# kyotovision-public/DRMNet

Measured on AMD Instinct MI355X. Metric: U-Net denoise steps/sec on 3x128x256 refmaps, higher is better.
Workload: dtype emulated fp32: f16 hi*hi + e4m3 cross terms (~15-bit products), fp32 acc; 1e-4 contract

## Files before the change

### drmnet_amd/_lib.py

```python
from __future__ import annotations

import ctypes as C
import os
from typing import Optional, Sequence

import torch

_HERE = os.path.dirname(os.path.abspath(__file__))
LIB_PATH = os.environ.get("DRM_LIB_PATH") or os.path.join(_HERE, "csrc", "libdrmnet_hip.so")
ABI_VERSION = 3
MAX_LEVELS = 8
LOSS_WORKSPACE_BYTES = 2048
DIFFUSION_LOSS_MAX_PARTS = 32
BRDF_ERROR_SUMS = 9
BRDF_ERROR_PARTS = 128


def diffusion_loss_workspace_bytes(B: int) -> int:
    return int(B) * DIFFUSION_LOSS_MAX_PARTS * 2 * 8


def brdf_error_workspace_bytes(C: int) -> int:
    return int(C) * BRDF_ERROR_PARTS * BRDF_ERROR_SUMS * 8


SYMBOLS = [
    "drm_abi_version", "drm_last_error",
    "drm_unet_create", "drm_unet_destroy", "drm_unet_param_count", "drm_unet_param_info", "drm_unet_load_params",
    "drm_unet_workspace_bytes", "drm_unet_forward",
    "drm_linear_forward", "drm_timestep_embedding", "drm_op_norm_act_conv", "drm_op_resblock", "drm_op_attention_block",
    "drm_drmnet_create", "drm_drmnet_destroy", "drm_drmnet_workspace_bytes", "drm_drmnet_set_batch_parts", "drm_drmnet_set_batch_part_min", "drm_drmnet_step", "drm_drmnet_sample",
    "drm_sampler_workspace_bytes", "drm_ddim_sample", "drm_ddim_sample_logged", "drm_ddpm_sample", "drm_ddim_sample_ex", "drm_ddpm_sample_ex", "drm_randn",
    "drm_profile_enable", "drm_profile_reset", "drm_profile_collect", "drm_unet_set_precision", "drm_set_op_precision",
    "drm_refmap_workspace_bytes", "drm_refmap_mask_make", "drm_erode_mask",
    "drm_unet_load_params_set", "drm_unet_use_set", "drm_set_graph_replay", "drm_set_upconv_split", "drm_graph_launches",
    "drm_map_chain", "drm_masked_log_range", "drm_luminance_scale", "drm_mirmap2envmap", "drm_hdr2ldr", "drm_resize", "drm_profile_variants",
    "drm_render_refmap", "drm_brdf_eval", "drm_render_refmap_views", "drm_validation_losses",
    "drm_render_refmap_lit", "drm_render_light_workspace_bytes",
    "drm_render_mesh_workspace_bytes", "drm_render_mesh",
    "drm_mesh_bvh_bytes", "drm_mesh_bvh_build", "drm_mesh_occluded", "drm_render_mesh_shadowed", "drm_render_mesh_lit",
    "drm_mesh_closest_hit", "drm_render_mesh_bounced",
    "drm_render_normals", "drm_image_from_refmap",
    "drm_brdf_to_merl", "drm_merl_eval", "drm_render_refmap_table", "drm_render_normals_table", "drm_brdf_error_sums",
    "drm_obs_forward_process", "drm_diffusion_losses",
    "drm_envmap2mirmap", "drm_rotate_envmap", "drm_mirimg2envmap", "drm_refmap2refimg",
]


class UNetDesc(C.Structure):
    _fields_ = [
# ... 118 lines not shown
    L.drm_ddpm_sample_ex.argtypes = [vp, fp, fp, fp, C.POINTER(C.c_float), i32, i32, fp, C.c_uint64, C.POINTER(SamplerOptions), i32, i32, i32, vp, C.c_size_t, vp]
    L.drm_randn.argtypes = [fp, C.c_size_t, C.c_uint64, C.c_uint64, vp]
    u8p = vp
    L.drm_refmap_workspace_bytes.argtypes = [C.c_int64, i32, C.c_float]
    L.drm_refmap_workspace_bytes.restype = C.c_size_t
    L.drm_refmap_mask_make.argtypes = [fp, fp, C.c_int64, i32, i32, C.c_float, i32, fp, u8p, vp, C.c_size_t, vp]
    L.drm_erode_mask.argtypes = [u8p, i32, i32, i32, u8p, vp]
    L.drm_unet_set_precision.argtypes = [vp, i32]
    L.drm_set_op_precision.argtypes = [i32]
    L.drm_profile_enable.argtypes = [i32]
    L.drm_profile_enable.restype = None
    L.drm_profile_reset.restype = None
    L.drm_profile_collect.argtypes = [C.POINTER(C.c_double), C.POINTER(C.c_double), C.POINTER(C.c_double), C.POINTER(C.c_int64)]
    L.drm_set_graph_replay.argtypes = [i32]
    L.drm_set_upconv_split.argtypes = [i32]
    L.drm_graph_launches.restype = C.c_int64
    L.drm_map_chain.argtypes = [fp, fp, C.c_int64, i32, C.POINTER(C.c_int32), C.POINTER(C.c_float), i32, fp, fp, fp, vp]
    L.drm_masked_log_range.argtypes = [fp, fp, i32, i32, i32, fp, fp, vp]
    L.drm_luminance_scale.argtypes = [fp, i32, i32, C.c_float, fp, vp]
    L.drm_mirmap2envmap.argtypes = [fp, fp, fp, i32, i32, i32, i32, i32, i32, i32, i32, vp]
    L.drm_hdr2ldr.argtypes = [fp, u8p, i32, C.c_float, C.c_float, fp, vp]
    L.drm_resize.argtypes = [fp, fp, i32, i32, i32, i32, i32, i32, vp]
    L.drm_profile_variants.argtypes = [C.c_char_p, C.c_size_t]
    L.drm_profile_variants.restype = C.c_size_t
    L.drm_render_refmap.argtypes = [fp, fp, fp, i32, i32, i32, i32, i32, i32, i32, vp]
    L.drm_brdf_eval.argtypes = [fp, i32, fp, fp, fp, fp, C.c_int64, vp]
    L.drm_render_refmap_views.argtypes = [fp, i32, fp, fp, fp, i32, i32, i32, i32, i32, i32, i32, vp]
    L.drm_render_refmap_lit.argtypes = [fp, i32, fp, fp, fp, i32, i32, i32, i32, i32, i32, i32, i32, vp, C.c_size_t, vp]
    L.drm_render_light_workspace_bytes.argtypes = [i32, i32, i32, i32]
    L.drm_render_light_workspace_bytes.restype = C.c_size_t
# ... 77 lines not shown
```

### drmnet_amd/csrc/abi.hip

```cpp
#include <atomic>
#include <cstring>
#include <memory>

#include "bvh.h"
#include "profiler.h"
#include "samplers.h"

using namespace drm;

struct drm_unet {
  UNet net;
};
struct drm_drmnet {
  DrmnetSampler s;
};

namespace {

int make_arena(Arena& ar, void* ws, size_t bytes, size_t need) {
  if (need == 0) return DRM_ERR_INVALID;
  if (bytes < need || ws == nullptr) {
    set_error("workspace too small: need " + std::to_string(need) + " bytes, got " + std::to_string(bytes));
    return DRM_ERR_WORKSPACE;
  }
// ... 409 lines not shown
    DRM_REQUIRE(precision_valid(precision),
                "precision must be 0 (fp32 MFMA), 1 (split fp16 x3), 2 (plain fp16 operands), 3 (split fp16 with fp8 cross terms) or 4 (plain bf16 operands)");
    g_op_precision.store(precision, std::memory_order_relaxed);
    return DRM_OK;
  });
}

int drm_set_upconv_split(int mode) {
  return guarded([&]() -> int {
    DRM_REQUIRE(mode >= 0 && mode <= 2, "upconv split mode: 0 = never, 1 = by the measured rule, 2 = wherever the form applies");
    set_upconv_split(mode);
    return DRM_OK;
  });
}

int drm_set_graph_replay(int on) {
  set_graph_replay(on != 0);
  return DRM_OK;
}
int64_t drm_graph_launches(void) { return (int64_t)graph_launches(); }

void drm_profile_enable(int on) { prof_enable(on); }
void drm_profile_reset(void) { prof_reset(); }
int drm_profile_collect(double* ms, double* flops, double* bytes, int64_t* launches) {
  return guarded([&]() -> int {
    DRM_REQUIRE(ms && flops && bytes && launches, "null argument");
    prof_collect(ms, flops, bytes, launches);
    return DRM_OK;
  });
}
// ... 279 lines not shown
```

### drmnet_amd/csrc/common.h

```cpp
#pragma once
#include <hip/hip_runtime.h>
#include <stdint.h>
#include <stdio.h>
#include <atomic>
#include <string>
#include "conv_forms.h"
#include "gn_fold.h"

namespace drm {

void set_error(const std::string& msg);
const char* last_error();

#define DRM_OK 0
#define DRM_ERR_INVALID 1
#define DRM_ERR_HIP 2
#define DRM_ERR_WORKSPACE 3
#define DRM_ERR_STATE 4

#define DRM_HIP_CHECK(expr)                                                                              \
  do {                                                                                                   \
    hipError_t _e = (expr);                                                                              \
    if (_e != hipSuccess) {                                                                              \
      ::drm::set_error(std::string(#expr) + " failed: " + hipGetErrorString(_e) + " at " + __FILE__ + ":" + \
// ... 37 lines not shown
struct XcdRange { int start, count; };
__host__ __device__ __forceinline__ XcdRange xcd_range(int total, int xcd) {
  const int q8 = total >> 3, r8 = total & 7;
  return {xcd < r8 ? xcd * (q8 + 1) : r8 * (q8 + 1) + (xcd - r8) * q8, q8 + (xcd < r8 ? 1 : 0)};
}


struct ConvArgs {
  const float* src0 = nullptr;
  const float* src1 = nullptr;
  int C0 = 0, C1 = 0, up0 = 0;
  int N = 0, H = 0, W = 0;
  const float* gn_scale = nullptr;
  const float* gn_shift = nullptr;
  int silu = 0;
  const float* w = nullptr;
  const float* bias = nullptr;
  int taps = 9;
  int Cout = 0;
  const float* emb = nullptr;
  int emb_stride = 0;
  const float* res = nullptr;
  float* out = nullptr;
  int out_nchw = 0, cout_valid = 0;
  int cin_real = 0;
  int ksplit = 1;
  size_t split_stride = 0;
  float* split_ws = nullptr;
  unsigned* tile_ticket = nullptr;
  int terms = 3;
// ... 26 lines not shown
struct ConvPlan {
  ConvKernel kernel = CONV_NONE;
  int terms = 0;
  ConvTile tile = TILE_128x32;
  int th = 0, tw = 0;
  bool ragged = false;
  int kc = 32;
  int ksplit = 1;
  SplitFinish finish = SPLIT_NONE;
  size_t tickets = 0;
  bool pool = false;
  bool gn_fold = false;
  bool split() const { return kernel == CONV_PIPELINE && terms != 0; }
};
ConvPlan plan_conv(const ConvArgs& a, int precision, bool want_pool = false, bool gn_foldable = false);
bool conv_split_weights(int precision, int cin);
int launch_conv(const ConvArgs& a, const ConvPlan& p, hipStream_t s);
template <int TAPS, int TERMS> int dispatch_s2(const ConvArgs& a, const ConvPlan& p, hipStream_t s);
int no_form(const ConvPlan& p);
size_t packed_conv_weight_split_floats(int taps, int CoutP, int CinP);
int launch_pack_conv_weight_split(const float* w, float* packed, float* scales, unsigned* scratch, int Cout, int Cin, int taps, int CoutP,
                                  int CinP, hipStream_t s, bool mx = false, bool bf16 = false);
enum Precision { PREC_FP32 = 0, PREC_F16X3 = 1, PREC_F16 = 2, PREC_F16MX = 3, PREC_BF16 = 4 };
inline bool precision_valid(int p) { return p >= PREC_FP32 && p <= PREC_BF16; }
inline int precision_terms(int p) { return p == PREC_F16 ? 1 : (p == PREC_BF16 ? 4 : (p == PREC_FP32 ? 0 : 3)); }
int launch_pack_conv_weight(const float* w, float* packed, int Cout, int Cin, int taps, int CoutP, int CinP, hipStream_t s);
int pack_conv_image(int precision, const float* w, float* packed, float* scale, unsigned* scratch, int Cout, int Cin, int taps, int CoutP, int CinP,
                    bool mx_site, hipStream_t s);
int launch_fold_upconv_weight(const float* w, float* wa, float* wb, int Cout, int C0, int C1, hipStream_t s);
int launch_fold_attn_params(const float* qkv_w, const float* qkv_b, const float* proj_w, const float* proj_b, float* w_out, float* b_out, int C,
// ... 139 lines not shown
```

### drmnet_amd/csrc/conv_plan.hip

```cpp
#include <algorithm>
#include "common.h"

namespace drm {

constexpr long long S2_MIN_WIDE_TILES = 176;
constexpr int GN_FOLD_MAX_N = 4;
bool conv_split_weights(int precision, int cin) { return precision != PREC_FP32 && cin % 32 == 0; }

static PixelTile conv_tile_family(int H, int W, bool pipeline) {
  auto area = [&](const PixelTile& f) { return (long long)((H + f.th - 1) / f.th * f.th) * ((W + f.tw - 1) / f.tw * f.tw); };
  const PixelTile* best = nullptr;
  for (const PixelTile& f : PIXEL_TILES)
    if (f.th * f.tw <= 128 && (!pipeline || pixel_tile_ragged(f.th, f.tw)) && (!best || area(f) < area(*best))) best = &f;
  return *best;
}

ConvPlan plan_conv(const ConvArgs& a, int precision, bool want_pool, bool gn_foldable) {
  ConvPlan p;
  const int Ctot = a.C0 + a.C1, hw = a.H * a.W;
  const bool split = precision != PREC_FP32, chunks = Ctot % 32 == 0 && a.C0 % 32 == 0;
  const long long rows = (long long)a.N * hw;
  auto wgs = [&](int bm, int bn) { return ((rows + bm - 1) / bm) * (a.Cout / bn); };
  if (a.w_img_stride_f4 != 0) {
    if (!split || a.H % 16 != 0 || a.W % 16 != 0 || a.Cout % 128 != 0 || Ctot % 128 != 0) return p;
// ... 41 lines not shown
  } else if (a.Cout % 64 == 0 && wgs(128, 64) >= 256) {
    tile(TILE_128x64, false);
  } else {
    tile(TILE_128x32, false);
  }
  p.ksplit = wide;
  if (wide == 1 && p.tile == TILE_128x32 && !a.out_nchw && a.w_img_stride_f4 == 0)
    p.ksplit = (int)std::max<long long>(std::min<long long>(std::min<long long>(8, Ctot / 32 / 4), 640 / std::max<long long>(wgs(128, 32), 1)), 1);
  if (p.ksplit > 1) {
    p.finish = (hw >= 128 && wide == 1) ? SPLIT_IN_LAUNCH : SPLIT_REDUCE;
    if (p.finish == SPLIT_IN_LAUNCH) p.tickets = ((size_t)a.N * hw / 128 + (size_t)hw / 16 + 2) * (size_t)(a.Cout / 32);
  }
  return p;
}

}
```

### drmnet_amd/csrc/conv_split2.hip

```cpp
#include <algorithm>
#include <utility>
#include <vector>
#include <cstdio>
#include <string>

#include "common.h"
#include "conv_epilogue.h"
#include "profiler.h"

#ifdef DRM_S2_STAMP
#define S2_STAMP(id)                                                                               \
  do {                                                                                             \
    if (stamp_on && stamp_n < 120) {                                                               \
      unsigned long long t_;                                                                       \
      __builtin_amdgcn_sched_barrier(0);                                                           \
      asm volatile("s_memtime %0\n\ts_waitcnt lgkmcnt(0)" : "=s"(t_)::"memory");                   \
      __builtin_amdgcn_sched_barrier(0);                                                           \
      if (lane == 0) {                                                                             \
        stamp_lds[(wave * 120 + stamp_n) * 2] = (unsigned)(id);                                    \
        stamp_lds[(wave * 120 + stamp_n) * 2 + 1] = (unsigned)t_;                                  \
      }                                                                                            \
      ++stamp_n;                                                                                   \
    }                                                                                              \
  } while (0)
// ... 126 lines not shown
               : "=&s"(keep)
               : "v"(voff), "s"(sbase), "s"(lds_dst)
               : "memory");
}
__device__ __forceinline__ void glds16(const void* gsrc, unsigned lds_dst) {
  unsigned keep;
  asm volatile("s_mov_b32 %0, m0\n\ts_mov_b32 m0, %2\n\ts_nop 0\n\tglobal_load_lds_dwordx4 %1, off\n\ts_mov_b32 m0, %0"
               : "=&s"(keep)
               : "v"(gsrc), "s"(lds_dst)
               : "memory");
}

__device__ __forceinline__ void gload16x2(f32x4& d0, f32x4& d1, const void* p) {
  asm volatile("global_load_dwordx4 %0, %2, off\n\tglobal_load_dwordx4 %1, %2, off offset:16" : "=&v"(d0), "=&v"(d1) : "v"(p) : "memory");
}
__device__ __forceinline__ void tie_regs(f32x4& x0, f32x4& x1) { asm volatile("" : "+v"(x0), "+v"(x1)::"memory"); }
__device__ __forceinline__ void tie_reg(f32x4& x) { asm volatile("" : "+v"(x)::"memory"); }

template <int... I, typename F>
__device__ __forceinline__ void static_for(std::integer_sequence<int, I...>, F&& f) {
  (f(std::integral_constant<int, I>{}), ...);
}

struct TilePos {
  int n0, ty0, tx0, co0;
  long long wofs;
};

template <int TAPS, int TH, int TW, int WM, int WN, int MT, int NT, int R, int TPS, int TERMS = 3, bool RAG = false, bool SK = false, bool POOL = false>
__global__ __launch_bounds__(WM* WN * 64, 2) void conv_split2_kernel(ConvArgs a) {
  using C = S2Cfg<TAPS, TH, TW, WM, WN, MT, NT, R, TPS, TERMS>;
  static_assert(!POOL || (C::SUB48 && C::TN == 1 && !RAG && !SK), "pooled output: one-image tiles of 4 x 8 patches");
  extern __shared__ float4 lds[];
  float4* As = lds;
  float4* Bs = lds + C::A_F4;
  double* lst = reinterpret_cast<double*>(lds + C::A_F4 + R * C::G_F4);
  [[maybe_unused]] double* lst2 = lst + C::TN * C::BN * 2;

#ifndef DRM_NO_KERNARG_TOUCH
  {
    typedef const __attribute__((address_space(4))) int* kptr_t;
    kptr_t ka = (kptr_t)__builtin_amdgcn_kernarg_segment_ptr();
    int touch = 0;
#pragma unroll
    for (int o = 0; o < (int)sizeof(ConvArgs); o += 64) touch ^= __builtin_nontemporal_load(ka + o / 4);
    asm volatile("" ::"s"(touch));
  }
// ... 232 lines not shown
  }
#pragma unroll
  for (int c = 0; c < NT; ++c) b_base[c] = (wn * NT + c) * 32 + r;

  f32x16 acc[MT][NT];
#pragma unroll
  for (int i = 0; i < MT; ++i)
#pragma unroll
    for (int c = 0; c < NT; ++c)
#pragma unroll
      for (int e = 0; e < 16; ++e) acc[i][c][e] = 0.f;

  const float inv_scale = a.w_inv_scale ? *a.w_inv_scale : 1.0f;
  constexpr int PPI = TH * TW;
  const bool st = a.stat_out != nullptr;
  if (st) {
    for (int k = tid; k < C::TN * C::BN * 2; k += C::NTHR) lst[k] = 0.0;
  }
  if constexpr (POOL) {
    for (int k = tid; k < C::TN * C::BN * 2; k += C::NTHR) lst2[k] = 0.0;
  }

  int gseq = 0;
  {
    int k2 = k_tile;
    TilePos tp = cur;
    int gi = 0;
#pragma unroll
    for (int G = 0; G < R - 1; ++G) {
      if (gi >= NGT) {
// ... 168 lines not shown
      gi = gi0 + (R - 1);
      co0 = cur.wofs;
      if (gi >= NGT) {
        gi -= NGT;
        if (gi >= NGT) gi %= NGT;
        co0 = nxt.wofs;
      }
    };
    auto issue_ahead = [&](int gi0) {
      int gi;
      long long co0;
      group_ahead(gi0, gi, co0);
      issue_G(gseq, gi, co0);
      ++gseq;
    };
    if constexpr (TAPS == 1) {
      for (int chunk = 0; chunk < nchunks; ++chunk) {
        const bool n1 = (chunk + 1 < nchunks) || has_next;
        const bool n2 = (chunk + 2 < nchunks) || (has_next && nchunks >= 2);
        auto side = [&]() {
          S2_STAMP(40);
          if (n1) {
            if (step == 0) wait_vmcnt<0>();
            else wait_vmcnt<C::G_PER>();
            S2_STAMP(41);
            store_A(As + ((step + 1) & 1) * C::A1_F4);
            S2_STAMP(42);
          }
          if (n2) {
            if (chunk + 2 < nchunks) load_A(cur, chunk + 2);
// ... 220 lines not shown
        const bool abl_noload = a.stamp_block & 0x200000;
#else
        constexpr bool abl_noload = false;
#endif
        if (a.res && first && !abl_noload) {
#pragma unroll
          for (int e = 0; e < 16; ++e) rv[e] = a.res[(pixb[e >> 2] + (e & 3)) * a.Cout + co];
        } else {
#pragma unroll
          for (int e = 0; e < 16; ++e) rv[e] = 0.f;
        }
        float s0 = 0.f, q0 = 0.f, s1 = 0.f, q1 = 0.f;
        float v[16];
#pragma unroll
        for (int e = 0; e < 16; ++e) {
          v[e] = epi_value(acc[i][c][e] * sv[e >> 2], bias, ev[e >> 2], rv[e]);
          acc[i][c][e] = 0.f;
        }
        const float p0 = okg[0] ? v[0] : (okg[1] ? v[4] : 0.f), p1 = okg[2] ? v[8] : (okg[3] ? v[12] : 0.f);
#pragma unroll
        for (int e = 0; e < 16; ++e) {
#ifdef DRM_S2_STAMP
          if (a.stamp_block & 0x100000) continue;
#endif
          if (okg[e >> 2]) {
            const float dv = v[e] - (e < 8 ? p0 : p1);
            if (e < 8) {
              s0 += dv;
              q0 += dv * dv;
            } else {
              s1 += dv;
// ... 255 lines not shown
    S2_STAMP(10);
    if (!has_next) break;
    k_tile += J;
    cur = nxt;
  }
  wait_vmcnt<0>();
#ifdef DRM_S2_STAMP
  if (a.stamp_out && (int)blockIdx.x == (a.stamp_block & 0xFFFF)) {
    asm volatile("s_waitcnt lgkmcnt(0)" ::: "memory");
    __builtin_amdgcn_s_barrier();
    for (int k = tid; k < C::NW * 240; k += C::NTHR) a.stamp_out[k] = stamp_lds[k];
  }
#endif
}

template <int TAPS, int TH, int TW, int WM, int WN, int MT, int NT, int R, int TPS, int TERMS = 3, bool RAG = false, bool SK = false, bool POOL = false>
static int launch_s2(const ConvArgs& a, hipStream_t s) {
  using C = S2Cfg<TAPS, TH, TW, WM, WN, MT, NT, R, TPS, TERMS>;
  constexpr auto kern = conv_split2_kernel<TAPS, TH, TW, WM, WN, MT, NT, R, TPS, TERMS, RAG, SK, POOL>;
  DRM_REQUIRE(RAG || (a.H % TH == 0 && a.W % TW == 0), "conv tile does not divide the map");
  DRM_REQUIRE(POOL == (a.pool_out != nullptr), "pooled output: only launches plan_conv pools");
  DRM_REQUIRE(!POOL || (a.pool_stat && a.stat_out && a.ksplit <= 1 && !a.out_nchw), "pooled output: needs both statistics tables, no split-K");
  if constexpr (TAPS == 4) {
    static_assert(!RAG && !SK && !POOL, "the parity form has no ragged, split-K or pooled instantiation");
    DRM_REQUIRE(!a.bias && !a.emb && !a.res && !a.stat_out && !a.out_nchw && a.ksplit <= 1 && !a.gnf.mom0 && !a.in_inv && a.w_img_stride_f4 == 0,
                "parity (4-tap) conv: weight un-scaling only -- no bias, emb, residual, statistics, split-K or GroupNorm fold");
    DRM_REQUIRE(a.C1 == 0 && !a.up0 && a.Cout % 4 == 0 && (a.Cout / 4) % C::BN == 0, "parity (4-tap) conv: one stored source, a Cout tile inside one parity");
  }
  const size_t lds_bytes = (size_t)(C::LDS_F4 + (POOL ? C::ST_F4 : 0)) * sizeof(float4);
  static_assert((C::LDS_F4 + (POOL ? C::ST_F4 : 0)) * 16 <= 160 * 1024, "LDS budget");
  const DeviceInfo* di = device_info();
  if (!di) return DRM_ERR_STATE;
  DRM_TRY(opt_in_lds<kern>(lds_bytes, di));
  const int groups = (a.N + C::TN - 1) / C::TN;
  const long long tiles = (long long)groups * ((a.H + TH - 1) / TH) * ((a.W + TW - 1) / TW) * (a.Cout / C::BN);
  DRM_REQUIRE(tiles > 0 && tiles < (1ll << 31), "conv grid size");
  const int per_cu = std::max(1, std::min((int)(di->lds_per_cu / lds_bytes), 8 / C::NW));
  long long grid = (long long)di->cus * per_cu;
  const int ngt = ((a.C0 + a.C1) / C::KC) * C::NG;
  const int ks = a.ksplit > 1 ? a.ksplit : 1;
  constexpr bool FUSE = SK;
  DRM_REQUIRE(ks == 1 || (!a.out_nchw && a.split_stride > 0 && a.w_img_stride_f4 == 0 && ((a.C0 + a.C1) / C::KC) / ks >= 1 && ks <= 8 &&
                          (a.split_ws ? (FUSE && a.tile_ticket != nullptr) : !a.stat_out)),
              "split-K launch contract");
  if (tiles < grid || ngt < R - 1 || (TAPS == 1 && ngt < 2) || ks > 1) grid = tiles;
  {
    prof_tag(a.N, a.H, a.W, a.C0 + a.C1, a.Cout);
    if (prof_enabled()) {
      static const std::string vname = [] {
        char b[192];
        snprintf(b, sizeof b, "void drm::conv_split2_kernel<%d, %d, %d, %d, %d, %d, %d, %d, %d, %d, %s, %s, %s>", TAPS, TH, TW, WM, WN, MT, NT, R, TPS, TERMS,
                 RAG ? "true" : "false", SK ? "true" : "false", POOL ? "true" : "false");
        return std::string(b);
      }();
      prof_variant(vname.c_str());
    }
    DRM_REQUIRE(a.w_img_stride_f4 == 0 || (C::TN == 1 && ks == 1), "per-image weights need one image per tile (H*W a multiple of the 256-pixel tile)");
    const ConvWork work = conv_work(a, TAPS);
    ProfScope ps(a.prof_kind == PROF_KINDS ? -1 : (a.prof_kind >= 0 ? a.prof_kind : (TAPS != 1 ? PROF_CONV3 : PROF_CONV1)), work.flops, work.bytes, s);
#ifdef DRM_S2_STAMP
    static const char* stamp_file = getenv("DRM_S2_STAMP_FILE");
    if (stamp_file && lds_bytes + 7680 <= di->lds_per_cu) {
      static unsigned* dbuf = nullptr;
      if (!dbuf) DRM_HIP_CHECK(hipMalloc(reinterpret_cast<void**>(&dbuf), 8192));
      DRM_HIP_CHECK(hipMemsetAsync(dbuf, 0, 8192, s));
      ConvArgs at = a;
// ... 18 lines not shown
      ConvArgs at = a;
      at.stamp_block = atoi(fl) & ~0xFFFF;
      hipLaunchKernelGGL(kern, dim3((unsigned)grid, (unsigned)ks), dim3(C::NTHR), lds_bytes, s, at);
    } else
#endif
    hipLaunchKernelGGL(kern, dim3((unsigned)grid, (unsigned)ks), dim3(C::NTHR), lds_bytes, s, a);
  }
  DRM_HIP_CHECK(hipGetLastError());
  return DRM_OK;
}

template <int TAPS, int TERMS, int TH, int TW, ConvTile T, bool RAG, bool SK, bool POOL>
static int launch_s2_form(const ConvArgs& a, const ConvPlan& p, hipStream_t s) {
  constexpr S2Form f = s2_form(TAPS, TERMS, TH, TW, T, RAG, SK, POOL);
  constexpr TileShape t = tile_shape(T);
  if constexpr (f.exists) return launch_s2<TAPS, TH, TW, t.wm, t.wn, t.mt, t.nt, f.ring, f.tps, TERMS, RAG, SK, POOL>(a, s);
  return no_form(p);
}

template <int TAPS, int TERMS, int TH, int TW, ConvTile T>
static int launch_s2_variant(const ConvArgs& a, const ConvPlan& p, hipStream_t s) {
  if (p.ragged) return launch_s2_form<TAPS, TERMS, TH, TW, T, true, false, false>(a, p, s);
  if (p.pool) return launch_s2_form<TAPS, TERMS, TH, TW, T, false, false, true>(a, p, s);
  if (p.finish == SPLIT_IN_LAUNCH) return launch_s2_form<TAPS, TERMS, TH, TW, T, false, true, false>(a, p, s);
  return launch_s2_form<TAPS, TERMS, TH, TW, T, false, false, false>(a, p, s);
}

template <int TAPS, int TERMS, int TH, int TW>
static int launch_s2_tile(const ConvArgs& a, const ConvPlan& p, hipStream_t s) {
#define DRM_X(name, wm, wn, mt, nt) if (p.tile == name) return launch_s2_variant<TAPS, TERMS, TH, TW, name>(a, p, s);
  DRM_CONV_TILES(DRM_X)
// ... 16 lines not shown
```

### drmnet_amd/csrc/engine.h

```cpp
#pragma once
#include <map>
#include <string>
#include <tuple>
#include <vector>

#include "../../include/drmnet_hip.h"
#include "common.h"

namespace drm {

struct Arena {
  char* base = nullptr;
  size_t cap = 0, off = 0, peak = 0;
  bool dry = false;
  bool failed = false;
  void* alloc_bytes(size_t bytes) {
    const size_t a = (off + 255) & ~size_t(255);
    off = a + bytes;
    if (off > peak) peak = off;
    if (dry) return nullptr;
    if (off > cap) {
      failed = true;
      return nullptr;
    }
// ... 127 lines not shown
  int dry_forward(int N, int H, int W, Arena& probe);
  ~UNet();
};

struct Ctx {
  Arena* ar;
  hipStream_t s;
  int N;
  int precision = PREC_FP32;
  bool dry() const { return ar->dry; }
  bool split() const { return precision == PREC_F16X3 || precision == PREC_F16 || precision == PREC_F16MX || precision == PREC_BF16; }
  int terms() const { return precision_terms(precision); }
};
Act new_act(Ctx& c, int C, int H, int W);
void set_upconv_split(int mode);
inline bool upconv_split_packable(int c0, int c1, int cout) { return c0 > 0 && c1 > 0 && c0 % 32 == 0 && c1 % 32 == 0 && cout % 32 == 0; }
int ensure_moments(Ctx& c, Act& a);
int expect_raw_sums(Ctx& c, Act& a);
int run_resblock(Ctx& c, const float* wbuf, const ResLayer& r, Act& x0, Act* x1, const float* emb_all, int emb_stride, Act& out, Act* pool = nullptr,
                 bool* pooled = nullptr);
int run_attention(Ctx& c, const float* wbuf, const AttnLayer& a, Act& x, Act& out);
int run_conv(Ctx& c, ConvArgs& a, const ConvPlan& p, const float* wbuf, size_t scale_off, Act* stats_for = nullptr);
int raw_input_guard(Ctx& c, ConvArgs& a, const ConvPlan& p, Act* x0, int lo0, int hi0, Act* x1, const unsigned* absmax_bits, int Ctab, int absmax_parts = 1);
int gn_params(Ctx& c, Act& x0, Act* x1, const float* gamma, const float* beta, float* scale, float* shift, ConvArgs* guard_for = nullptr,
              ConvArgs* fold_into = nullptr);

}
```

### drmnet_amd/csrc/engine.hip

```cpp
#include "engine.h"

#include <algorithm>
#include <atomic>
#include <deque>
#include <mutex>

namespace drm {

static thread_local std::string g_err;
void set_error(const std::string& msg) { g_err = msg; }
const char* last_error() { return g_err.c_str(); }

const DeviceInfo* device_info() {
  constexpr int MAX_DEV = 64;
  static DeviceInfo info[MAX_DEV];
  static std::atomic<int> state[MAX_DEV];
  int dev = 0;
  if (hipGetDevice(&dev) != hipSuccess || dev < 0 || dev >= MAX_DEV) {
    set_error("device_info: no current HIP device");
    return nullptr;
  }
  int st = state[dev].load(std::memory_order_acquire);
  if (st == 0) {
    static std::mutex mu;
// ... 405 lines not shown
  const int mode = g_upconv_split.load(std::memory_order_relaxed);
  if (mode == 0 || !r.up_c0 || !x0.up || !x1 || x0.C != r.up_c0 || !upconv_split_packable(x0.C, x1->C, r.cout)) return u;
  auto plain = [](const ConvPlan& p) { return p.kernel == CONV_PIPELINE && !p.ragged && p.ksplit == 1 && !p.gn_fold && !p.pool; };
  if (!plain(pa)) return u;
  u.a4.C0 = x0.C; u.a4.N = a.N; u.a4.H = a.H >> 1; u.a4.W = a.W >> 1; u.a4.taps = 4; u.a4.Cout = 4 * r.cout; u.a4.mx_site = 1;
  u.b9.C0 = x1->C; u.b9.N = a.N; u.b9.H = a.H; u.b9.W = a.W; u.b9.taps = 9; u.b9.Cout = r.cout; u.b9.mx_site = 1;
  u.p4 = plan_conv(u.a4, c.precision);
  u.p9 = plan_conv(u.b9, c.precision);
  if (!plain(u.p4) || !plain(u.p9)) return u;
  if (r.cout % tile_shape(u.p4.tile).bn() != 0) return u;
  if (mode == 1 && (u.p4.tile > TILE_256x128 || u.p9.tile > TILE_256x128)) return u;
  u.on = true;
  return u;
}

int run_resblock(Ctx& c, const float* Wb, const ResLayer& r, Act& x0, Act* x1, const float* emb_all, int emb_stride, Act& out, Act* pool, bool* pooled) {
  DRM_TRY(arena_ok(c));
  const int H = x0.H, W = x0.W;
  const int C0 = x0.C, C1 = x1 ? x1->C : 0;
  DRM_REQUIRE(C0 + C1 == r.cin, "resblock input channels");
  DRM_REQUIRE(!x1 || (x1->H == H && x1->W == W && !x1->up), "resblock skip tensor shape");
  DRM_REQUIRE(r.has_skip || (!x1 && !x0.up), "identity skip on a concatenated / upsampled input is not supported");
  const size_t mark = c.ar->mark();
  float* sc1 = c.ar->alloc<float>((size_t)c.N * r.cin);
  float* sh1 = c.ar->alloc<float>((size_t)c.N * r.cin);
  Act h1 = new_act(c, r.cout, H, W);
  float* sc2 = c.ar->alloc<float>((size_t)c.N * r.cout);
  float* sh2 = c.ar->alloc<float>((size_t)c.N * r.cout);
  ConvArgs k;
  ConvArgs a;
  a.src0 = x0.p; a.src1 = x1 ? x1->p : nullptr; a.C0 = C0; a.C1 = C1; a.up0 = x0.up;
  a.N = c.N; a.H = H; a.W = W; a.taps = 9; a.Cout = r.cout; a.mx_site = 1;
  const ConvPlan pa = plan_conv(a, c.precision, false, true);
  ConvPlan pk;
  if (r.has_skip) {
    k.C0 = C0; k.C1 = C1; k.N = c.N; k.H = H; k.W = W; k.taps = 1; k.Cout = r.cout;
    pk = plan_conv(k, c.precision);
  }
  DRM_TRY(gn_params(c, x0, x1, Wb + r.n1_w, Wb + r.n1_b, sc1, sh1, pk.split() ? &k : nullptr, pa.gn_fold ? &a : nullptr));
  splitk_workspace(c, a, pa);
  UpconvSplit up = plan_upconv_split(c, r, a, pa, x0, x1);
  if (up.on) {
    if (!c.dry()) {
      ConvArgs& a4 = up.a4;
      a4.src0 = x0.p; a4.gn_scale = sc1; a4.gn_shift = sh1; a4.gn_ld = r.cin; a4.silu = 1;
      a4.w = Wb + r.c1a_w; a4.out = h1.p;
      DRM_TRY(run_conv(c, a4, up.p4, Wb, r.c1a_s, nullptr));
      ConvArgs& b9 = up.b9;
      b9.src0 = x1->p; b9.gn_scale = sc1 + x0.C; b9.gn_shift = sh1 + x0.C; b9.gn_ld = r.cin; b9.silu = 1;
      b9.w = Wb + r.c1b_w; b9.bias = Wb + r.c1_b;
      b9.emb = emb_all ? emb_all + r.emb_off : nullptr; b9.emb_stride = emb_stride;
      b9.res = h1.p; b9.out = h1.p;
      DRM_TRY(run_conv(c, b9, up.p9, Wb, r.c1b_s, &h1));
    }
  } else if (!c.dry()) {
// ... 2 lines not shown
    a.emb = emb_all ? emb_all + r.emb_off : nullptr; a.emb_stride = emb_stride;
    a.out = h1.p;
    DRM_TRY(run_conv(c, a, pa, Wb, r.c1_s, &h1));
  }
  ConvArgs b;
  b.src0 = h1.p; b.C0 = r.cout; b.N = c.N; b.H = H; b.W = W; b.taps = 9; b.Cout = r.cout; b.mx_site = 1;
  const ConvPlan pb = plan_conv(b, c.precision, pool != nullptr, true);
  DRM_TRY(gn_params(c, h1, nullptr, Wb + r.n2_w, Wb + r.n2_b, sc2, sh2, nullptr, pb.gn_fold ? &b : nullptr));
  splitk_workspace(c, b, pb);
  if (pooled) *pooled = pb.pool;
  if (pb.pool) DRM_TRY(expect_raw_sums(c, *pool));
  if (r.has_skip) splitk_workspace(c, k, pk);
  if (!c.dry()) {
    const float* res = x0.p;
    if (r.has_skip) {
      k.src0 = x0.p; k.src1 = x1 ? x1->p : nullptr; k.up0 = x0.up;
      k.w = Wb + r.sk_w; k.bias = Wb + r.sk_b;
      k.out = out.p;
      DRM_TRY(run_conv(c, k, pk, Wb, r.sk_s, nullptr));
      res = out.p;
    }
    b.gn_scale = sc2; b.gn_shift = sh2; b.silu = 1;
    b.w = Wb + r.c2_w; b.bias = Wb + r.c2_b;
    b.res = res; b.out = out.p;
    if (pb.pool) {
      b.pool_out = pool->p;
      b.pool_stat = pool->mom;
    }
    DRM_TRY(run_conv(c, b, pb, Wb, r.c2_s, &out));
  }
  c.ar->release(mark);
  return DRM_OK;
}

// ... 222 lines not shown
```

### drmnet_amd/ops.py

```python
from __future__ import annotations

from typing import Optional, Sequence

import torch

from . import _lib


def set_precision(precision: str) -> None:
    modes = {"fp32": 0, "f16x3": 1, "f16": 2, "f16mx": 3, "bf16": 4}
    if precision not in modes:
        raise ValueError(f"precision must be one of {list(modes)}")
    _lib.check(_lib.lib().drm_set_op_precision(modes[precision]))


def set_graph_replay(on: bool) -> None:
    _lib.check(_lib.lib().drm_set_graph_replay(int(bool(on))))


def set_upconv_split(mode: int) -> None:
    _lib.check(_lib.lib().drm_set_upconv_split(int(mode)))


UPCONV_TAP_GROUPS = {0: {0: (0,), 1: (1, 2)}, 1: {0: (0, 1), 1: (2,)}}


def fold_upconv_weight(w: torch.Tensor, c0: int):
    cout = w.shape[0]
    w0 = w[:, :c0].double()
    wa = torch.zeros((4, cout, c0, 2, 2), dtype=torch.float64, device=w.device)
    for a in (0, 1):
        for b in (0, 1):
            for dy in (0, 1):
                for dx in (0, 1):
                    for ky in UPCONV_TAP_GROUPS[a][dy]:
                        for kx in UPCONV_TAP_GROUPS[b][dx]:
# ... 380 lines not shown
```

### include/drmnet_hip.h

```cpp
#ifndef DRMNET_HIP_H
#define DRMNET_HIP_H

#include <stddef.h>
#include <stdint.h>

#ifdef __cplusplus
extern "C" {
#endif

#define DRM_ABI_VERSION 3
#define DRM_MAX_LEVELS 8

int drm_abi_version(void);
const char* drm_last_error(void);

typedef struct drm_unet_desc {
  int32_t kind;
  int32_t in_channels;
  int32_t model_channels;
  int32_t out_channels;
  int32_t num_res_blocks;
  int32_t n_levels;
  int32_t channel_mult[DRM_MAX_LEVELS];
  int32_t n_attn;
// ... 87 lines not shown
  const float* dropout_keep;
} drm_sampler_options;

int drm_ddim_sample_ex(drm_unet* net, float* x, const float* cond, const int64_t* timesteps, const float* coef, int S, int num_steps,
                       const float* noise, uint64_t seed, const drm_sampler_options* opt, int log_every_t, float* log_x, float* log_pred_x0, int log_slots,
                       int32_t* n_logged, int N, int H, int W, void* workspace, size_t workspace_bytes, void* stream);
int drm_ddpm_sample_ex(drm_unet* net, float* x, float* pred_x0, const float* cond, const float* coef, int T_start, int clip_denoised,
                       const float* noise, uint64_t seed, const drm_sampler_options* opt, int N, int H, int W, void* workspace, size_t workspace_bytes,
                       void* stream);

size_t drm_sampler_workspace_bytes(const drm_unet* net, int N, int H, int W);

int drm_set_graph_replay(int on);

int drm_set_upconv_split(int mode);
int64_t drm_graph_launches(void);

#define DRM_PROFILE_KINDS 5
void drm_profile_enable(int on);
void drm_profile_reset(void);
int drm_profile_collect(double* ms, double* flops, double* bytes, int64_t* launches);
size_t drm_profile_variants(char* buf, size_t cap);

int drm_randn(float* out, size_t n, uint64_t seed, uint64_t offset, void* stream);

size_t drm_refmap_workspace_bytes(int64_t n, int res, float angle_threshold);
int drm_refmap_mask_make(const float* colors, const float* normals, int64_t n, int channels, int res, float angle_threshold, int min_points,
                         float* refmap, uint8_t* refmask, void* workspace, size_t workspace_bytes, void* stream);

int drm_erode_mask(const uint8_t* mask, int H, int W, int kernel_size, uint8_t* out, void* stream);
// ... 114 lines not shown
```

Baseline: 883.6.

## Compute upsampled half of decoder skip 1x1 conv at low resolution

For decoder resblocks whose 1x1 skip conv reads a nearest-upsampled source concatenated with a full-resolution source, the upsampled channels are now convolved at half resolution. Their raw accumulators are written to a slab. A second full-resolution 1x1 launch over the other source preloads those accumulators at the upsampled position before adding its own products and the bias. This removes the redundant three quarters of the MACs on the upsampled channels. In exchange it adds a kernel launch, a slab round trip through memory, and new template instantiations with a carried-accumulator path. It is on by default under a tile-size rule.

```diff
diff --git a/drmnet_amd/_lib.py b/drmnet_amd/_lib.py
--- a/drmnet_amd/_lib.py
+++ b/drmnet_amd/_lib.py
@@ -33,7 +33,7 @@
     "drm_sampler_workspace_bytes", "drm_ddim_sample", "drm_ddim_sample_logged", "drm_ddpm_sample", "drm_ddim_sample_ex", "drm_ddpm_sample_ex", "drm_randn",
     "drm_profile_enable", "drm_profile_reset", "drm_profile_collect", "drm_unet_set_precision", "drm_set_op_precision",
     "drm_refmap_workspace_bytes", "drm_refmap_mask_make", "drm_erode_mask",
-    "drm_unet_load_params_set", "drm_unet_use_set", "drm_set_graph_replay", "drm_set_upconv_split", "drm_graph_launches",
+    "drm_unet_load_params_set", "drm_unet_use_set", "drm_set_graph_replay", "drm_set_upconv_split", "drm_set_skip_lowres", "drm_graph_launches",
     "drm_map_chain", "drm_masked_log_range", "drm_luminance_scale", "drm_mirmap2envmap", "drm_hdr2ldr", "drm_resize", "drm_profile_variants",
     "drm_render_refmap", "drm_brdf_eval", "drm_render_refmap_views", "drm_validation_losses",
     "drm_render_refmap_lit", "drm_render_light_workspace_bytes",
@@ -182,6 +182,7 @@
     L.drm_profile_collect.argtypes = [C.POINTER(C.c_double), C.POINTER(C.c_double), C.POINTER(C.c_double), C.POINTER(C.c_int64)]
     L.drm_set_graph_replay.argtypes = [i32]
     L.drm_set_upconv_split.argtypes = [i32]
+    L.drm_set_skip_lowres.argtypes = [i32]
     L.drm_graph_launches.restype = C.c_int64
     L.drm_map_chain.argtypes = [fp, fp, C.c_int64, i32, C.POINTER(C.c_int32), C.POINTER(C.c_float), i32, fp, fp, fp, vp]
     L.drm_masked_log_range.argtypes = [fp, fp, i32, i32, i32, fp, fp, vp]
diff --git a/drmnet_amd/csrc/abi.hip b/drmnet_amd/csrc/abi.hip
--- a/drmnet_amd/csrc/abi.hip
+++ b/drmnet_amd/csrc/abi.hip
@@ -447,6 +447,14 @@
   });
 }
 
+int drm_set_skip_lowres(int mode) {
+  return guarded([&]() -> int {
+    DRM_REQUIRE(mode >= 0 && mode <= 2, "skip lowres mode: 0 = never, 1 = by the measured rule, 2 = wherever the form is legal");
+    set_skip_lowres(mode);
+    return DRM_OK;
+  });
+}
+
 int drm_set_graph_replay(int on) {
   set_graph_replay(on != 0);
   return DRM_OK;
diff --git a/drmnet_amd/csrc/common.h b/drmnet_amd/csrc/common.h
--- a/drmnet_amd/csrc/common.h
+++ b/drmnet_amd/csrc/common.h
@@ -75,6 +75,7 @@
   const float* gn_scale = nullptr;
   const float* gn_shift = nullptr;
   int silu = 0;
+  int acc_io = 0;
   const float* w = nullptr;
   const float* bias = nullptr;
   int taps = 9;
@@ -131,6 +132,12 @@
   bool split() const { return kernel == CONV_PIPELINE && terms != 0; }
 };
 ConvPlan plan_conv(const ConvArgs& a, int precision, bool want_pool = false, bool gn_foldable = false);
+struct SkipLowres {
+  bool on = false;
+  ConvArgs ka, kb;
+  ConvPlan pa, pb;
+};
+SkipLowres plan_skip_lowres(const ConvArgs& k, const ConvPlan& pk, int precision, int mode);
 bool conv_split_weights(int precision, int cin);
 int launch_conv(const ConvArgs& a, const ConvPlan& p, hipStream_t s);
 template <int TAPS, int TERMS> int dispatch_s2(const ConvArgs& a, const ConvPlan& p, hipStream_t s);
diff --git a/drmnet_amd/csrc/conv_plan.hip b/drmnet_amd/csrc/conv_plan.hip
--- a/drmnet_amd/csrc/conv_plan.hip
+++ b/drmnet_amd/csrc/conv_plan.hip
@@ -79,4 +79,23 @@
   return p;
 }
 
+static bool skip_lowres_rule(const SkipLowres& u) { return u.pa.tile <= TILE_256x128 && u.pb.tile <= TILE_256x128; }
+
+SkipLowres plan_skip_lowres(const ConvArgs& k, const ConvPlan& pk, int precision, int mode) {
+  SkipLowres u;
+  if (mode == 0 || k.taps != 1 || k.C0 <= 0 || k.C1 <= 0 || k.C0 % 32 != 0 || k.C1 % 32 != 0 || k.H % 2 != 0 || k.W % 2 != 0 || k.out_nchw ||
+      k.w_img_stride_f4 != 0)
+    return u;
+  auto plain = [](const ConvPlan& p) { return p.kernel == CONV_PIPELINE && !p.ragged && p.ksplit == 1 && !p.gn_fold && !p.pool; };
+  if (!plain(pk)) return u;
+  u.ka.C0 = k.C0; u.ka.N = k.N; u.ka.H = k.H >> 1; u.ka.W = k.W >> 1; u.ka.taps = 1; u.ka.Cout = k.Cout;
+  u.kb.C0 = k.C1; u.kb.N = k.N; u.kb.H = k.H; u.kb.W = k.W; u.kb.taps = 1; u.kb.Cout = k.Cout;
+  u.pa = plan_conv(u.ka, precision);
+  u.pb = plan_conv(u.kb, precision);
+  if (!plain(u.pa) || !plain(u.pb) || u.pa.terms != pk.terms || u.pb.terms != pk.terms) return u;
+  if (mode == 1 && !skip_lowres_rule(u)) return u;
+  u.on = true;
+  return u;
 }
+
+}
diff --git a/drmnet_amd/csrc/conv_split2.hip b/drmnet_amd/csrc/conv_split2.hip
--- a/drmnet_amd/csrc/conv_split2.hip
+++ b/drmnet_amd/csrc/conv_split2.hip
@@ -164,6 +164,7 @@
 __device__ __forceinline__ void gload16x2(f32x4& d0, f32x4& d1, const void* p) {
   asm volatile("global_load_dwordx4 %0, %2, off\n\tglobal_load_dwordx4 %1, %2, off offset:16" : "=&v"(d0), "=&v"(d1) : "v"(p) : "memory");
 }
+__device__ __forceinline__ void gload16(f32x4& d, const void* p) { asm volatile("global_load_dwordx4 %0, %1, off" : "=&v"(d) : "v"(p) : "memory"); }
 __device__ __forceinline__ void tie_regs(f32x4& x0, f32x4& x1) { asm volatile("" : "+v"(x0), "+v"(x1)::"memory"); }
 __device__ __forceinline__ void tie_reg(f32x4& x) { asm volatile("" : "+v"(x)::"memory"); }
 
@@ -177,10 +178,14 @@
   long long wofs;
 };
 
-template <int TAPS, int TH, int TW, int WM, int WN, int MT, int NT, int R, int TPS, int TERMS = 3, bool RAG = false, bool SK = false, bool POOL = false>
+constexpr int S2_ACC = 10;
+template <int TAPS, int TH, int TW, int WM, int WN, int MT, int NT, int R, int TPS, int TERMS_ = 3, bool RAG = false, bool SK = false, bool POOL = false>
 __global__ __launch_bounds__(WM* WN * 64, 2) void conv_split2_kernel(ConvArgs a) {
+  constexpr int TERMS = TERMS_ % S2_ACC;
+  constexpr bool ACC_IO = TERMS_ >= S2_ACC;
   using C = S2Cfg<TAPS, TH, TW, WM, WN, MT, NT, R, TPS, TERMS>;
   static_assert(!POOL || (C::SUB48 && C::TN == 1 && !RAG && !SK), "pooled output: one-image tiles of 4 x 8 patches");
+  static_assert(!ACC_IO || (TAPS == 1 && !RAG && !SK && !POOL), "carried accumulators: the plain 1x1 forms");
   extern __shared__ float4 lds[];
   float4* As = lds;
   float4* Bs = lds + C::A_F4;
@@ -443,6 +448,7 @@
   const float inv_scale = a.w_inv_scale ? *a.w_inv_scale : 1.0f;
   constexpr int PPI = TH * TW;
   const bool st = a.stat_out != nullptr;
+  [[maybe_unused]] const bool acc_raw = ACC_IO && a.acc_io == 1;
   if (st) {
     for (int k = tid; k < C::TN * C::BN * 2; k += C::NTHR) lst[k] = 0.0;
   }
@@ -641,6 +647,37 @@
       issue_G(gseq, gi, co0);
       ++gseq;
     };
+    if constexpr (ACC_IO) {
+      if (a.acc_io == 2) {
+        const float* const acc_in = a.split_ws;
+        f32x4 t[MT][NT][4];
+        const int Hh = a.H >> 1, Wh = a.W >> 1;
+#pragma unroll
+        for (int i = 0; i < MT; ++i)
+#pragma unroll
+          for (int g = 0; g < 4; ++g) {
+            const int row = (wm * MT + i) * 32 + 8 * g + 4 * h;
+            int img, py, px;
+            C::rowmap(row, img, py, px);
+            const int n = min(cur.n0 + img, a.N - 1);
+            const size_t pp = ((size_t)n * Hh + ((cur.ty0 + py) >> 1)) * Wh + ((cur.tx0 + px + (r & 3)) >> 1);
+#pragma unroll
+            for (int c = 0; c < NT; ++c) gload16(t[i][c][g], acc_in + pp * a.Cout + cur.co0 + (wn * NT + c) * 32 + (r & ~3));
+          }
+        wait_vmcnt<0>();
+#pragma unroll
+        for (int i = 0; i < MT; ++i)
+#pragma unroll
+          for (int c = 0; c < NT; ++c)
+#pragma unroll
+            for (int g = 0; g < 4; ++g) {
+              tie_reg(t[i][c][g]);
+              float v0 = t[i][c][g].x, v1 = t[i][c][g].y, v2 = t[i][c][g].z, v3 = t[i][c][g].w;
+              quad_transpose(v0, v1, v2, v3, r);
+              acc[i][c][4 * g] = v0; acc[i][c][4 * g + 1] = v1; acc[i][c][4 * g + 2] = v2; acc[i][c][4 * g + 3] = v3;
+            }
+      }
+    }
     if constexpr (TAPS == 1) {
       for (int chunk = 0; chunk < nchunks; ++chunk) {
         const bool n1 = (chunk + 1 < nchunks) || has_next;
@@ -891,7 +928,8 @@
         float v[16];
 #pragma unroll
         for (int e = 0; e < 16; ++e) {
-          v[e] = epi_value(acc[i][c][e] * sv[e >> 2], bias, ev[e >> 2], rv[e]);
+          if constexpr (ACC_IO) v[e] = acc_raw ? acc[i][c][e] : epi_value(acc[i][c][e] * sv[e >> 2], bias, ev[e >> 2], rv[e]);
+          else v[e] = epi_value(acc[i][c][e] * sv[e >> 2], bias, ev[e >> 2], rv[e]);
           acc[i][c][e] = 0.f;
         }
         const float p0 = okg[0] ? v[0] : (okg[1] ? v[4] : 0.f), p1 = okg[2] ? v[8] : (okg[3] ? v[12] : 0.f);
@@ -1177,11 +1215,16 @@
 #endif
 }
 
-template <int TAPS, int TH, int TW, int WM, int WN, int MT, int NT, int R, int TPS, int TERMS = 3, bool RAG = false, bool SK = false, bool POOL = false>
+template <int TAPS, int TH, int TW, int WM, int WN, int MT, int NT, int R, int TPS, int TERMS = 3, bool RAG = false, bool SK = false, bool POOL = false, bool ACC = false>
 static int launch_s2(const ConvArgs& a, hipStream_t s) {
   using C = S2Cfg<TAPS, TH, TW, WM, WN, MT, NT, R, TPS, TERMS>;
-  constexpr auto kern = conv_split2_kernel<TAPS, TH, TW, WM, WN, MT, NT, R, TPS, TERMS, RAG, SK, POOL>;
+  constexpr auto kern = conv_split2_kernel<TAPS, TH, TW, WM, WN, MT, NT, R, TPS, ACC ? S2_ACC + TERMS : TERMS, RAG, SK, POOL>;
   DRM_REQUIRE(RAG || (a.H % TH == 0 && a.W % TW == 0), "conv tile does not divide the map");
+  DRM_REQUIRE(ACC == (a.acc_io != 0) && a.acc_io >= 0 && a.acc_io <= 2, "carried accumulators run on the S2_ACC instantiations, and nothing else does");
+  if constexpr (ACC)
+    DRM_REQUIRE(a.ksplit <= 1 && !a.out_nchw && a.w_img_stride_f4 == 0 && !a.gnf.mom0 && !a.up0 && a.C1 == 0 &&
+                    (a.acc_io == 1 ? (!a.bias && !a.emb && !a.res && !a.stat_out) : (a.split_ws && a.H % 2 == 0 && a.W % 2 == 0)),
+                "carried accumulators: a plain whole-tile 1x1 launch on one stored source (1: no epilogue terms; 2: the accumulators, an even map)");
   DRM_REQUIRE(POOL == (a.pool_out != nullptr), "pooled output: only launches plan_conv pools");
   DRM_REQUIRE(!POOL || (a.pool_stat && a.stat_out && a.ksplit <= 1 && !a.out_nchw), "pooled output: needs both statistics tables, no split-K");
   if constexpr (TAPS == 4) {
@@ -1212,7 +1255,7 @@
     if (prof_enabled()) {
       static const std::string vname = [] {
         char b[192];
-        snprintf(b, sizeof b, "void drm::conv_split2_kernel<%d, %d, %d, %d, %d, %d, %d, %d, %d, %d, %s, %s, %s>", TAPS, TH, TW, WM, WN, MT, NT, R, TPS, TERMS,
+        snprintf(b, sizeof b, "void drm::conv_split2_kernel<%d, %d, %d, %d, %d, %d, %d, %d, %d, %d, %s, %s, %s>", TAPS, TH, TW, WM, WN, MT, NT, R, TPS, ACC ? S2_ACC + TERMS : TERMS,
                  RAG ? "true" : "false", SK ? "true" : "false", POOL ? "true" : "false");
         return std::string(b);
       }();
@@ -1261,7 +1304,12 @@
 static int launch_s2_form(const ConvArgs& a, const ConvPlan& p, hipStream_t s) {
   constexpr S2Form f = s2_form(TAPS, TERMS, TH, TW, T, RAG, SK, POOL);
   constexpr TileShape t = tile_shape(T);
-  if constexpr (f.exists) return launch_s2<TAPS, TH, TW, t.wm, t.wn, t.mt, t.nt, f.ring, f.tps, TERMS, RAG, SK, POOL>(a, s);
+  if constexpr (f.exists) {
+    if constexpr (TAPS == 1 && !RAG && !SK && !POOL) {
+      if (a.acc_io) return launch_s2<TAPS, TH, TW, t.wm, t.wn, t.mt, t.nt, f.ring, f.tps, TERMS, false, false, false, true>(a, s);
+    }
+    return launch_s2<TAPS, TH, TW, t.wm, t.wn, t.mt, t.nt, f.ring, f.tps, TERMS, RAG, SK, POOL>(a, s);
+  }
   return no_form(p);
 }
 
diff --git a/drmnet_amd/csrc/engine.h b/drmnet_amd/csrc/engine.h
--- a/drmnet_amd/csrc/engine.h
+++ b/drmnet_amd/csrc/engine.h
@@ -165,6 +165,7 @@
 };
 Act new_act(Ctx& c, int C, int H, int W);
 void set_upconv_split(int mode);
+void set_skip_lowres(int mode);
 inline bool upconv_split_packable(int c0, int c1, int cout) { return c0 > 0 && c1 > 0 && c0 % 32 == 0 && c1 % 32 == 0 && cout % 32 == 0; }
 int ensure_moments(Ctx& c, Act& a);
 int expect_raw_sums(Ctx& c, Act& a);
diff --git a/drmnet_amd/csrc/engine.hip b/drmnet_amd/csrc/engine.hip
--- a/drmnet_amd/csrc/engine.hip
+++ b/drmnet_amd/csrc/engine.hip
@@ -443,6 +443,9 @@
   return u;
 }
 
+static std::atomic<int> g_skip_lowres{1};
+void set_skip_lowres(int mode) { g_skip_lowres.store(mode); }
+
 int run_resblock(Ctx& c, const float* Wb, const ResLayer& r, Act& x0, Act* x1, const float* emb_all, int emb_stride, Act& out, Act* pool, bool* pooled) {
   DRM_TRY(arena_ok(c));
   const int H = x0.H, W = x0.W;
@@ -468,6 +471,22 @@
   }
   DRM_TRY(gn_params(c, x0, x1, Wb + r.n1_w, Wb + r.n1_b, sc1, sh1, pk.split() ? &k : nullptr, pa.gn_fold ? &a : nullptr));
   splitk_workspace(c, a, pa);
+  SkipLowres sl;
+  if (r.has_skip && x0.up && x1) sl = plan_skip_lowres(k, pk, c.precision, g_skip_lowres.load(std::memory_order_relaxed));
+  float* sl_slab = !sl.on ? nullptr : (pa.gn_fold ? c.ar->alloc<float>((size_t)c.N * (H >> 1) * (W >> 1) * r.cout) : h1.p);
+  auto skip_lowres = [&]() -> int {
+    DRM_TRY(arena_ok(c));
+    ConvArgs& ka = sl.ka;
+    ka.src0 = x0.p; ka.gn_scale = k.gn_scale; ka.gn_shift = k.gn_shift; ka.gn_ld = r.cin; ka.in_inv = k.in_inv;
+    ka.w = Wb + r.sk_w; ka.out = sl_slab; ka.acc_io = 1;
+    DRM_TRY(run_conv(c, ka, sl.pa, Wb, r.sk_s, nullptr));
+    ConvArgs& kb = sl.kb;
+    kb.src0 = x1->p; kb.gn_scale = k.gn_scale ? k.gn_scale + C0 : nullptr; kb.gn_shift = k.gn_shift ? k.gn_shift + C0 : nullptr; kb.gn_ld = r.cin;
+    kb.in_inv = k.in_inv;
+    kb.w = Wb + r.sk_w + (size_t)C0 * r.cout; kb.bias = Wb + r.sk_b; kb.out = out.p; kb.acc_io = 2; kb.split_ws = sl_slab;
+    return run_conv(c, kb, sl.pb, Wb, r.sk_s, nullptr);
+  };
+  if (sl.on && !pa.gn_fold && !c.dry()) DRM_TRY(skip_lowres());
   UpconvSplit up = plan_upconv_split(c, r, a, pa, x0, x1);
   if (up.on) {
     if (!c.dry()) {
@@ -500,10 +519,14 @@
   if (!c.dry()) {
     const float* res = x0.p;
     if (r.has_skip) {
-      k.src0 = x0.p; k.src1 = x1 ? x1->p : nullptr; k.up0 = x0.up;
-      k.w = Wb + r.sk_w; k.bias = Wb + r.sk_b;
-      k.out = out.p;
-      DRM_TRY(run_conv(c, k, pk, Wb, r.sk_s, nullptr));
+      if (sl.on) {
+        if (pa.gn_fold) DRM_TRY(skip_lowres());
+      } else {
+        k.src0 = x0.p; k.src1 = x1 ? x1->p : nullptr; k.up0 = x0.up;
+        k.w = Wb + r.sk_w; k.bias = Wb + r.sk_b;
+        k.out = out.p;
+        DRM_TRY(run_conv(c, k, pk, Wb, r.sk_s, nullptr));
+      }
       res = out.p;
     }
     b.gn_scale = sc2; b.gn_shift = sh2; b.silu = 1;
diff --git a/drmnet_amd/ops.py b/drmnet_amd/ops.py
--- a/drmnet_amd/ops.py
+++ b/drmnet_amd/ops.py
@@ -20,6 +20,10 @@
 
 def set_upconv_split(mode: int) -> None:
     _lib.check(_lib.lib().drm_set_upconv_split(int(mode)))
+
+
+def set_skip_lowres(mode: int) -> None:
+    _lib.check(_lib.lib().drm_set_skip_lowres(int(mode)))
 
 
 UPCONV_TAP_GROUPS = {0: {0: (0,), 1: (1, 2)}, 1: {0: (0, 1), 1: (2,)}}
diff --git a/include/drmnet_hip.h b/include/drmnet_hip.h
--- a/include/drmnet_hip.h
+++ b/include/drmnet_hip.h
@@ -125,6 +125,7 @@
 int drm_set_graph_replay(int on);
 
 int drm_set_upconv_split(int mode);
+int drm_set_skip_lowres(int mode);
 int64_t drm_graph_launches(void);
 
 #define DRM_PROFILE_KINDS 5
```

Measured after the change: 888.2, median of 6. Within noise of the previous version (+0.5%).
